# megvii-research/Far3D

Measured on AMD Instinct MI355X. Metric: samples/sec (7-cam frame) end-to-end @ VoV-99 640x960, higher is better.
Workload: dtype bf16x3; 1 GPU; BASELINE configs[1]: 7 cameras 3x640x960, VoV-99, A=1544 queries (644 learned + 644 adaptive + 256 propagated), 2312 self-attn keys, 6 decoder layers, streaming memory on, ego motion on; proposals=topk, fused_rows=True, parallelism=single GPU, weights=seeded random (far3d_amd.weights.init_state_dict, seed 0)

## Files before the change

### far3d_amd/csrc/conv_ws.hip

```cpp
#include "conv_ws.hpp"

#ifdef FAR3D_PROFILING
std::atomic<int> g_ws_ablate{0};
extern "C" int far3d_conv_ws_set_ablate(int mask) { g_ws_ablate.store(mask); return 0; }
#endif

int far3d_conv_ws_launch(const IgemmParams& P, int tile, hipStream_t st) {
  switch (tile) {
    case 400: return launch_conv3x3_ws<2, 4, 2, 2, 4, true, true>(P, st);
    case 401: return launch_conv3x3_ws<1, 8, 2, 1, 4, true, true>(P, st);
    case 402: return launch_conv3x3_ws<1, 8, 5, 1, 4, true, false>(P, st);
    case 403: return launch_conv3x3_ws<2, 4, 3, 1, 4, true, true>(P, st);
    case 404: return launch_conv3x3_ws<2, 2, 1, 2, 2, true, true>(P, st);
    case 405: return launch_conv3x3_ws<2, 4, 2, 1, 4, true, true>(P, st);
    case 406: return launch_conv3x3_ws<2, 4, 1, 2, 4, true, true>(P, st);
    case 407: return launch_conv3x3_ws<1, 4, 5, 1, 2, true, false>(P, st);
    case 408: return launch_conv3x3_ws<1, 4, 3, 1, 2, true, true>(P, st);
    case 409: return launch_conv3x3_ws<2, 4, 2, 2, 2, true, true>(P, st);
    case 410: return launch_conv3x3_ws<2, 4, 2, 2, 4, true, true, 4>(P, st);
    case 411: return launch_conv3x3_ws<2, 4, 2, 1, 4, true, true, 6>(P, st);
    case 412: return launch_conv3x3_ws<2, 4, 1, 2, 4, true, true, 8>(P, st);
    case 413: return launch_conv3x3_ws<1, 8, 2, 1, 4, true, true, 8>(P, st);
    case 414: return launch_conv3x3_ws<1, 4, 5, 1, 2, true, false, 5>(P, st);
    case 415: return launch_conv3x3_ws<2, 2, 1, 2, 2, true, true, 6>(P, st);
    case 416: return launch_conv3x3_ws<2, 4, 3, 1, 4, true, true, 4>(P, st);
    case 417: return launch_conv3x3_ws<2, 4, 2, 1, 4, true, true, 4>(P, st);
    case 418: return launch_conv3x3_ws<4, 2, 2, 2, 4, true, true, 3>(P, st);
    case 419: return launch_conv3x3_ws<4, 2, 2, 1, 4, true, true, 3>(P, st);
    case 440: return launch_conv3x3_ws<2, 4, 2, 2, 4, true, true, 3, true>(P, st);
    case 444: return launch_conv3x3_ws<2, 2, 1, 2, 2, true, true, 3, true>(P, st);
    case 445: return launch_conv3x3_ws<2, 4, 2, 1, 4, true, true, 6, true>(P, st);
    case 450: return launch_conv3x3_ws<2, 4, 2, 1, 4, true, true, 6, false, 3>(P, st);
    case 451: return launch_conv3x3_ws<2, 4, 1, 2, 4, true, true, 6, false, 3>(P, st);
    case 452: return launch_conv3x3_ws<2, 4, 1, 2, 4, true, true, 9, false, 3>(P, st);
    case 453: return launch_conv3x3_ws<1, 8, 2, 1, 4, true, true, 6, false, 3>(P, st);
    case 454: return launch_conv3x3_ws<1, 8, 2, 1, 4, true, true, 9, false, 3>(P, st);
    case 455: return launch_conv3x3_ws<1, 7, 2, 1, 4, true, true, 9, false, 3>(P, st);
    case 456: return launch_conv3x3_ws<2, 7, 1, 1, 2, true, true, 9, false, 3>(P, st);
    case 457: return launch_conv3x3_ws<2, 2, 1, 2, 2, true, true, 6, false, 3>(P, st);
    case 458: return launch_conv3x3_ws<1, 4, 3, 1, 2, true, true, 6, false, 3>(P, st);
    case 459: return launch_conv3x3_ws<2, 4, 1, 1, 4, true, true, 9, false, 3>(P, st);
    case 420: return launch_conv3x3_ws<2, 4, 2, 2, 4, false, true>(P, st);
    case 421: return launch_conv3x3_ws<1, 8, 2, 1, 4, false, true>(P, st);
    case 422: return launch_conv3x3_ws<1, 8, 5, 1, 4, false, true>(P, st);
    case 423: return launch_conv3x3_ws<2, 4, 3, 1, 4, false, true>(P, st);
    default: break;
  }
  far3d_set_error("far3d_conv2d_nhwc: unknown wave-specialised tile %d", tile);
  return FAR3D_ERR_ARG;
}

int far3d_gemm_ws_launch(const IgemmParams& P, int tile, hipStream_t st) {
  switch (tile) {
    case 460: return launch_gemm1x1_ws<4, 2, 1, 2, 4, 4, 1>(P, st);
    case 461: return launch_gemm1x1_ws<4, 2, 1, 2, 4, 4, 2>(P, st);
    case 462: return launch_gemm1x1_ws<2, 4, 2, 1, 4, 4, 2>(P, st);
    case 463: return launch_gemm1x1_ws<2, 2, 2, 2, 4, 4, 2>(P, st);
    case 464: return launch_gemm1x1_ws<4, 2, 2, 2, 4, 3, 1>(P, st);
    case 465: return launch_gemm1x1_ws<4, 2, 1, 2, 2, 4, 2>(P, st);
    case 466: return launch_gemm1x1_ws<2, 2, 1, 2, 4, 6, 3>(P, st);
    case 467: return launch_gemm1x1_ws<2, 4, 1, 1, 4, 6, 2>(P, st);
    case 468: return launch_gemm1x1_ws<2, 2, 1, 2, 2, 3, 1>(P, st);
    case 469: return launch_gemm1x1_ws<4, 2, 1, 2, 4, 2, 1>(P, st);
    case 470: return launch_gemm1x1_ws<2, 4, 2, 2, 4, 3, 1>(P, st);
    case 471: return launch_gemm1x1_ws<2, 2, 4, 2, 4, 3, 1>(P, st);
    case 473: return launch_gemm1x1_ws<4, 2, 2, 2, 2, 3, 1>(P, st);
    case 474: return launch_gemm1x1_ws<3, 2, 2, 2, 4, 3, 1>(P, st);
    case 475: return launch_gemm1x1_ws<2, 2, 2, 2, 4, 4, 1>(P, st);
    case 476: return launch_gemm1x1_ws<2, 4, 2, 2, 2, 3, 1>(P, st);
    default: break;
  }
  far3d_set_error("far3d_conv2d_nhwc: unknown wave-specialised GEMM tile %d", tile);
  return FAR3D_ERR_ARG;
}
```

### far3d_amd/csrc/conv_ws.hpp

```cpp
#pragma once
#include "igemm_kernels.hpp"
#include <type_traits>

__device__ __forceinline__ __amdgpu_buffer_rsrc_t uniform_rsrc(const void* p, long nbytes) {
  const unsigned long long a = (unsigned long long)(uintptr_t)p;
  const unsigned lo = __builtin_amdgcn_readfirstlane((unsigned)a), hi = __builtin_amdgcn_readfirstlane((unsigned)(a >> 32));
  const int nb = __builtin_amdgcn_readfirstlane((int)(nbytes < 0x7fffffffL ? nbytes : 0x7fffffffL));
  return __builtin_amdgcn_make_buffer_rsrc((void*)(uintptr_t)(((unsigned long long)hi << 32) | lo), 0, nb, 0x00020000);
}

__device__ __forceinline__ void wait_vmcnt_dyn(int n) {
#define FAR3D_WVC(k) case k: wait_vmcnt<k>(); break;
  switch (n) {
    FAR3D_WVC(0) FAR3D_WVC(1) FAR3D_WVC(2) FAR3D_WVC(3) FAR3D_WVC(4) FAR3D_WVC(5) FAR3D_WVC(6) FAR3D_WVC(7) FAR3D_WVC(8)
    FAR3D_WVC(9) FAR3D_WVC(10) FAR3D_WVC(11) FAR3D_WVC(12) FAR3D_WVC(13) FAR3D_WVC(14) FAR3D_WVC(15) FAR3D_WVC(16)
    FAR3D_WVC(17) FAR3D_WVC(18) FAR3D_WVC(19) FAR3D_WVC(20) FAR3D_WVC(21) FAR3D_WVC(22) FAR3D_WVC(23) FAR3D_WVC(24)
    FAR3D_WVC(25) FAR3D_WVC(26) FAR3D_WVC(27) FAR3D_WVC(28) FAR3D_WVC(29) FAR3D_WVC(30) FAR3D_WVC(31) FAR3D_WVC(32)
    FAR3D_WVC(33) FAR3D_WVC(34) FAR3D_WVC(35) FAR3D_WVC(36) FAR3D_WVC(37) FAR3D_WVC(38) FAR3D_WVC(39) FAR3D_WVC(40)
    FAR3D_WVC(41) FAR3D_WVC(42) FAR3D_WVC(43) FAR3D_WVC(44) FAR3D_WVC(45) FAR3D_WVC(46) FAR3D_WVC(47)
    default: wait_vmcnt<48>(); break;
  }
#undef FAR3D_WVC
}

#ifdef FAR3D_PROFILING
extern std::atomic<int> g_ws_ablate;
#define FAR3D_WS_ABLATE_ARG g_ws_ablate.load(std::memory_order_relaxed)
#else
#define FAR3D_WS_ABLATE_ARG 0
#endif

template <int WGM, int WGN, int WM, int WN, int NP, bool PAIR, bool DBUF, int NSW = 3, bool FLAGS = false, int GRP = 1>
__global__ __launch_bounds__(64 * (WGM * WGN + NP)) void conv3x3_ws_kernel(IgemmParams P, int tiles_x, int tiles_y, int n_mt, int n_items, int ablate) {
#if defined(__HIP_DEVICE_COMPILE__)
  constexpr int NWC = WGM * WGN;
  static_assert(NSW >= 3, "ring depth");
  static_assert(GRP == 1 || (GRP == 3 && (NSW == 6 || NSW == 9) && !FLAGS), "one barrier per tap, or per kernel row with a ring of 2 or 3 rows");
  constexpr int NG = NSW / GRP;
  constexpr int PLD = PAIR ? 2 : 1;
  constexpr int BM = 32 * WGM * WM, TH = WGN * WN, PW = 34, PH = TH + 2, PPIX = PW * PH;
  constexpr int PG = (PPIX + 15) / 16, PATCH_B = PG * 1024;
  constexpr int GA = BM / 16, WST = BM * 64, WSTAGE = PLD * WST;
  constexpr int PBASE = NSW * WSTAGE, PBUF = PLD * PATCH_B;
  constexpr int RB = WN + 2;
  constexpr int FLAGB = PBASE + 2 * PBUF;
  static_assert(FLAGB + (FLAGS ? 128 : 0) <= 163840, "LDS budget");
  static_assert(!FLAGS || (NP <= 4 && NWC <= 8), "flag words: one b128 read per 4 counters");
  extern __shared__ __attribute__((aligned(1024))) unsigned char smem[];
  [[maybe_unused]] volatile unsigned* const flg = reinterpret_cast<volatile unsigned*>(smem + FLAGB);
  if constexpr (FLAGS) {
    if (threadIdx.x < 32) flg[threadIdx.x] = 0u;
    __syncthreads();
  }
  [[maybe_unused]] bool gave_up = false;
  constexpr int SPIN_LIMIT = 1 << 18;
  const int t = threadIdx.x, lane = t & 63, wv = __builtin_amdgcn_readfirstlane(t >> 6);
  const int nchunks = P.cin_pad / 32;
  const int spt = 9 * nchunks;
  const int my_items = (n_items - (int)blockIdx.x + (int)gridDim.x - 1) / (int)gridDim.x;
  const int total_steps = my_items * spt, total_chunks = my_items * nchunks;
  const int Ktot = 9 * P.cin_pad * PLD;
#ifdef FAR3D_PROFILING
  if (P.prof && t == 0) {
    unsigned hw_, xcc_;
    asm volatile("s_getreg_b32 %0, hwreg(HW_REG_HW_ID)" : "=s"(hw_));
    asm volatile("s_getreg_b32 %0, hwreg(HW_REG_XCC_ID)" : "=s"(xcc_));
    P.prof[(long)blockIdx.x * 16 + 0] = (unsigned long long)hw_ | ((unsigned long long)xcc_ << 32);
    P.prof[(long)blockIdx.x * 16 + 6] = (unsigned long long)__builtin_amdgcn_s_memrealtime();
    P.prof[(long)blockIdx.x * 16 + 1] = (unsigned long long)__builtin_amdgcn_s_memtime();
    P.prof[(long)blockIdx.x * 16 + 4] = (unsigned long long)my_items;
  }
#endif

  if (wv >= NWC) {
    const int pw = wv - NWC;
    constexpr int GPL = (PG + NP - 1) / NP, GWL = (GA + NP - 1) / NP;
    const int rg = lane >> 2, pc = lane & 3;
    const int lc = pc ^ ((rg >> 2) & 3);
    int npq = (PG - pw + NP - 1) / NP, nwq = (GA - pw + NP - 1) / NP;
    npq = npq < 0 ? 0 : npq; nwq = nwq < 0 ? 0 : nwq;
    const int np = npq * PLD, nw = nwq * PLD;
    constexpr unsigned OOB = 0x80000000u;
    unsigned wvoff[GWL];
#pragma unroll
    for (int i = 0; i < GWL; ++i) wvoff[i] = (unsigned)((((pw + NP * i) * 16 + rg) * Ktot + lc * 8) * 2);
    const long img_bytes = (long)P.H * P.W * P.ldx * 2;
    unsigned pvoff[GPL];
    const bf16_t* x_base = nullptr;
    const bf16_t* w_base = nullptr;
    long w_bytes = 0;
    auto decode = [&](int k, int& n, int& y0, int& x0, int& m0) __attribute__((always_inline)) {
      const int item = (int)blockIdx.x + k * (int)gridDim.x;
      const int mt = item % n_mt, pt = item / n_mt;
      const int tx = pt % tiles_x, r = pt / tiles_x;
      const int ty = r % tiles_y;
      n = __builtin_amdgcn_readfirstlane(r / tiles_y); y0 = __builtin_amdgcn_readfirstlane(ty * TH);
      x0 = __builtin_amdgcn_readfirstlane(tx * 32); m0 = __builtin_amdgcn_readfirstlane(mt * BM);
    };
    auto set_w_tile = [&](int k) __attribute__((always_inline)) {
      int n, y0, x0, m0;
      decode(k, n, y0, x0, m0);
      w_base = reinterpret_cast<const bf16_t*>(P.w) + (long)m0 * Ktot;
      w_bytes = w_tile_bytes(BM, m0, P.Cout, Ktot);
    };
    auto set_p_tile = [&](int k) __attribute__((always_inline)) {
      int n, y0, x0, m0;
      decode(k, n, y0, x0, m0);
      x_base = reinterpret_cast<const bf16_t*>(P.x) + (long)n * P.x_img_stride;
#pragma unroll
      for (int i = 0; i < GPL; ++i) {
        const int idx = (pw + NP * i) * 16 + rg;
        const int py = idx / PW, px = idx - py * PW;
        const int iy = y0 - 1 + py, ix = x0 - 1 + px;
        const bool ok = idx < PPIX && iy >= 0 && iy < P.H && ix >= 0 && ix < P.W;
        pvoff[i] = ok ? (unsigned)((((long)iy * P.W + ix) * P.ldx + lc * 8) * 2) : OOB;
      }
    };
    auto issue_w = [&](int step_in_tile, int stage) __attribute__((always_inline)) {
      const int c = step_in_tile / 9, tap = step_in_tile - 9 * c;
      const int kb = __builtin_amdgcn_readfirstlane((tap * P.cin_pad + c * 32) * PLD * 2);
      const __amdgpu_buffer_rsrc_t rs_w = uniform_rsrc(w_base, w_bytes);
      const int sbase = __builtin_amdgcn_readfirstlane(stage * WSTAGE);
#pragma unroll
      for (int i = 0; i < GWL; ++i) {
        if (i < nwq) {
#pragma unroll
          for (int pl = 0; pl < PLD; ++pl)
            __builtin_amdgcn_raw_ptr_buffer_load_lds(rs_w, (lds_void_t*)(smem + sbase + pl * WST + (pw + NP * i) * 1024), 16, wvoff[i],
                                                     kb + pl * 64, 0, 0);
        }
      }
    };
    auto issue_p = [&](int chunk_in_tile, int buf) __attribute__((always_inline)) {
      const __amdgpu_buffer_rsrc_t rs_x = uniform_rsrc(x_base, img_bytes);
      const int pbase = __builtin_amdgcn_readfirstlane(PBASE + buf * PBUF), coff = __builtin_amdgcn_readfirstlane(chunk_in_tile * (64 * PLD));
#pragma unroll
      for (int i = 0; i < GPL; ++i) {
        if (i < npq) {
#pragma unroll
          for (int pl = 0; pl < PLD; ++pl)
            __builtin_amdgcn_raw_ptr_buffer_load_lds(rs_x, (lds_void_t*)(smem + pbase + pl * PATCH_B + (pw + NP * i) * 1024), 16, pvoff[i],
                                                     coff + pl * 64, 0, 0);
        }
      }
    };
    int sw_step = 0, sw_tile = 0, sw_stage = 0;
    int gp_chunk = 0, gp_tile = 0, gp_buf = 0;
    int w_left = total_steps, p_left = total_chunks;
    set_w_tile(0); set_p_tile(0);
    auto next_w = [&]() __attribute__((always_inline)) {
      if (!(ablate & 1)) issue_w(sw_step, sw_stage);
      --w_left;
      sw_stage = sw_stage == NSW - 1 ? 0 : sw_stage + 1;
      if (++sw_step == spt) { sw_step = 0; ++sw_tile; if (w_left > 0) set_w_tile(sw_tile); }
    };
    auto next_p = [&]() __attribute__((always_inline)) {
      if (!(ablate & 1)) issue_p(gp_chunk, gp_buf);
      --p_left;
      gp_buf ^= 1;
      if (++gp_chunk == nchunks) { gp_chunk = 0; ++gp_tile; if (p_left > 0) set_p_tile(gp_tile); }
    };
    next_p();
#pragma unroll
    for (int i = 0; i < (NG - 1) * GRP; ++i)
      if (w_left > 0) next_w();
    const int total_groups = total_steps / GRP, gpc = 9 / GRP;
    int gic = 0;
    unsigned phist = 0;
    for (int g = 0; g < total_groups; ++g) {
      int ahead = total_groups - 1 - g;
      ahead = ahead > NG - 2 ? NG - 2 : ahead;
      const int cnt = ahead * GRP * nw + __builtin_popcount(phist & ((1u << (NG - 1)) - 1u)) * np;
      const int S = g * GRP;
      if (ablate & 1) wait_vmcnt<0>(); else wait_vmcnt_dyn(cnt);
      if constexpr (FLAGS) {
        if (lane == 0) flg[pw] = (unsigned)(S + 1);
        if (S > 0 && !(ablate & 8)) {
          for (int spins = 0; !gave_up; ++spins) {
            const u32x4_t c0 = *reinterpret_cast<volatile u32x4_t*>(smem + FLAGB + 64);
            u32x4_t c1 = c0;
            if constexpr (NWC > 4) c1 = *reinterpret_cast<volatile u32x4_t*>(smem + FLAGB + 80);
            unsigned m = c0.x;
            if constexpr (NWC > 1) m = min(m, c0.y);
            if constexpr (NWC > 2) m = min(m, c0.z);
            if constexpr (NWC > 3) m = min(m, c0.w);
            if constexpr (NWC > 4) m = min(m, c1.x);
            if constexpr (NWC > 5) m = min(m, c1.y);
            if constexpr (NWC > 6) m = min(m, c1.z);
            if constexpr (NWC > 7) m = min(m, c1.w);
            if (__builtin_amdgcn_readfirstlane(m) >= (unsigned)S) break;
            if (spins > SPIN_LIMIT) gave_up = true;
            __builtin_amdgcn_s_sleep(2);
          }
        }
      } else {
#ifdef FAR3D_PROFILING
        if (!(ablate & 8))
#endif
        __builtin_amdgcn_s_barrier();
      }
      asm volatile("" ::: "memory");
#pragma unroll
      for (int i = 0; i < GRP; ++i)
        if (w_left > 0) next_w();
      phist <<= 1;
      if (gic == 0 && p_left > 0) { next_p(); phist |= 1u; }
      gic = gic == gpc - 1 ? 0 : gic + 1;
    }
    return;
  }

  const int wm = wv / WGN, wn = wv % WGN, l31 = lane & 31, hi = lane >> 5;
  int aaddr[WM], baddr[RB][3];
#pragma unroll
  for (int i = 0; i < WM; ++i) {
    const int r = (wm * WM + i) * 32 + l31;
    aaddr[i] = r * 64 + ((hi ^ ((r >> 2) & 3)) << 4);
  }
#pragma unroll
  for (int r = 0; r < RB; ++r)
#pragma unroll
    for (int kx = 0; kx < 3; ++kx) {
      const int idx = (wn * WN + r) * PW + l31 + kx;
      baddr[r][kx] = PBASE + idx * 64 + ((hi ^ ((idx >> 2) & 3)) << 4);
    }
  f32x16_t acc[WM][WN];
  u32x4_t fa[2][PLD][WM], fb[2][PLD][WN];

  auto load_a = [&](int set, int soff, int kk) __attribute__((always_inline)) {
#ifdef FAR3D_PROFILING
    if (ablate & 4) return;
#endif
    const int x32 = kk * 32;
#pragma unroll
    for (int pl = 0; pl < PLD; ++pl)
#pragma unroll
      for (int i = 0; i < WM; ++i) fa[set][pl][i] = *reinterpret_cast<const u32x4_t*>(smem + pl * WST + ((aaddr[i] ^ x32) + soff));
  };
  auto load_b = [&](int set, int tap, int kk) __attribute__((always_inline)) {
#ifdef FAR3D_PROFILING
    if (ablate & 4) return;
#endif
    const int ky = tap / 3, kx = tap - 3 * ky, x32 = kk * 32;
#pragma unroll
    for (int pl = 0; pl < PLD; ++pl)
#pragma unroll
      for (int j = 0; j < WN; ++j) fb[set][pl][j] = *reinterpret_cast<const u32x4_t*>(smem + pl * PATCH_B + (baddr[j + ky][kx] ^ x32));
  };
  auto load_set = [&](int set, int soff, int tap, int kk) __attribute__((always_inline)) { load_a(set, soff, kk); load_b(set, tap, kk); };
  auto mma_term = [&](int set, int term) __attribute__((always_inline)) {
    const int pa = (PAIR && term == 0) ? 1 : 0, pb = (PAIR && term == 1) ? 1 : 0;
#pragma unroll
    for (int i = 0; i < WM; ++i)
#pragma unroll
      for (int j = 0; j < WN; ++j) mma<bf16_t>(acc[i][j], fa[set][pa][i], fb[set][pb][j]);
  };
  auto mma_set = [&](int set) __attribute__((always_inline)) {
    if constexpr (PAIR) { mma_term(set, 0); mma_term(set, 1); }
    mma_term(set, 2);
  };

  int G = 0;
  int soff = 0;
  [[maybe_unused]] int Sg = 0;
  [[maybe_unused]] u32x4_t pfl = {0u, 0u, 0u, 0u};
#ifdef FAR3D_PROFILING
  unsigned long long pf_ta = 0, pf_tb = 0, pf_wait = 0, pf_body = 0, pf_epi = 0;
  const bool pf_on = P.prof != nullptr && wv == 0;
#endif
  for (int k = 0; k < my_items; ++k) {
    const int item = (int)blockIdx.x + k * (int)gridDim.x;
    const int mt = item % n_mt, pt = item / n_mt;
    const int tx = pt % tiles_x, rr = pt / tiles_x;
    const int ty = rr % tiles_y, n = rr / tiles_y;
    const int x0 = tx * 32, y0 = ty * TH, m0 = mt * BM;
#pragma unroll
    for (int i = 0; i < WM; ++i)
#pragma unroll
      for (int j = 0; j < WN; ++j)
#pragma unroll
        for (int r = 0; r < 16; ++r) acc[i][j][r] = 0.f;

    for (int c = 0; c < nchunks; ++c, ++G) {
#pragma unroll
      for (int tap = 0; tap < 9; ++tap) {
        const int stage = soff;
        if (tap % GRP == 0) {
        __builtin_amdgcn_s_waitcnt(0xc07f);
#ifdef FAR3D_PROFILING
        if (pf_on) {
          const unsigned long long now = __builtin_amdgcn_s_memtime();
          if (pf_tb) { pf_wait += pf_tb - pf_ta; pf_body += now - pf_tb; }
          pf_ta = now;
        }
#endif
        if constexpr (FLAGS) {
          if (lane == 0) flg[16 + wv] = (unsigned)Sg;
          if (!(ablate & 8)) {
            for (int spins = 0; !gave_up; ++spins) {
              unsigned m = pfl.x;
              if constexpr (NP > 1) m = min(m, pfl.y);
              if constexpr (NP > 2) m = min(m, pfl.z);
              if constexpr (NP > 3) m = min(m, pfl.w);
              if (__builtin_amdgcn_readfirstlane(m) >= (unsigned)(Sg + 1)) break;
              if (spins > SPIN_LIMIT) gave_up = true;
              __builtin_amdgcn_s_sleep(1);
              pfl = *reinterpret_cast<volatile u32x4_t*>(smem + FLAGB);
            }
          }
          ++Sg;
        } else {
#ifdef FAR3D_PROFILING
          if (!(ablate & 8))
#endif
          __builtin_amdgcn_s_barrier();
        }
        asm volatile("" ::: "memory");
        __builtin_amdgcn_sched_barrier(0);
#ifdef FAR3D_PROFILING
        if (pf_on) pf_tb = __builtin_amdgcn_s_memtime();
        if (tap == 0 && c == 0 && k == 0 && P.prof && t == 0) P.prof[(long)blockIdx.x * 16 + 2] = (unsigned long long)__builtin_amdgcn_s_memtime();
#endif
        }
        if (ablate & 2) { soff = soff == (NSW - 1) * WSTAGE ? 0 : soff + WSTAGE; continue; }
        if constexpr (DBUF) {
          load_set(0, stage, tap, 0);
          __builtin_amdgcn_sched_barrier(0);
          if (tap > 0 || c > 0) mma_set(1);
          __builtin_amdgcn_sched_barrier(0);
          load_a(1, stage, 1);
          if constexpr (FLAGS) pfl = *reinterpret_cast<volatile u32x4_t*>(smem + FLAGB);
          __builtin_amdgcn_sched_barrier(0);
          if constexpr (PAIR) {
            mma_term(0, 0);
            __builtin_amdgcn_sched_barrier(0);
            load_b(1, tap, 1);
            __builtin_amdgcn_sched_barrier(0);
            mma_term(0, 1);
            mma_term(0, 2);
          } else {
            load_b(1, tap, 1);
            __builtin_amdgcn_sched_barrier(0);
            mma_term(0, 2);
          }
          __builtin_amdgcn_sched_barrier(0);
          soff = soff == (NSW - 1) * WSTAGE ? 0 : soff + WSTAGE;
        } else {
          load_set(0, stage, tap, 0);
          __builtin_amdgcn_sched_barrier(0);
          mma_set(0);
          __builtin_amdgcn_sched_barrier(0);
          load_set(0, stage, tap, 1);
          if constexpr (FLAGS) pfl = *reinterpret_cast<volatile u32x4_t*>(smem + FLAGB);
          __builtin_amdgcn_sched_barrier(0);
          mma_set(0);
          __builtin_amdgcn_sched_barrier(0);
          soff = soff == (NSW - 1) * WSTAGE ? 0 : soff + WSTAGE;
        }
      }
      const int d = (G & 1) ? -PBUF : PBUF;
#pragma unroll
      for (int r = 0; r < RB; ++r)
#pragma unroll
        for (int kx = 0; kx < 3; ++kx) baddr[r][kx] += d;
    }
    if constexpr (DBUF) mma_set(1);
    __builtin_amdgcn_sched_barrier(0);
#ifdef FAR3D_PROFILING
    unsigned long long pf_e0 = 0;
    if (pf_on) {
      pf_e0 = __builtin_amdgcn_s_memtime();
      if (pf_tb) { pf_wait += pf_tb - pf_ta; pf_body += pf_e0 - pf_tb; pf_tb = 0; }
    }
#endif

    {
      const int px = x0 + l31;
      unsigned char* yb = reinterpret_cast<unsigned char*>(P.y);
#pragma unroll
      for (int j = 0; j < WN; ++j) {
        const int py = y0 + wn * WN + j;
        const bool ok = py < P.Ho && px < P.Wo;
        const long pix_b = ((long)n * P.y_img_stride + ((long)py * P.Wo + px) * P.ldy) * 2;
#pragma unroll
        for (int i = 0; i < WM; ++i) {
          const int cb = m0 + (wm * WM + i) * 32;
          if (cb >= P.Cout) continue;
#pragma unroll
          for (int qp = 0; qp < 2; ++qp) {
            uint2 h[2], l[2];
#pragma unroll
            for (int u = 0; u < 2; ++u) {
              const int q = 2 * qp + u;
              float4 b4 = make_float4(0.f, 0.f, 0.f, 0.f);
              if (P.bias) b4 = *reinterpret_cast<const float4*>(P.bias + cb + 8 * q + 4 * hi);
              float v[4];
#pragma unroll
              for (int e = 0; e < 4; ++e) v[e] = acc[i][j][4 * q + e];
              v[0] += b4.x; v[1] += b4.y; v[2] += b4.z; v[3] += b4.w;
              if (P.act == ACT_RELU) {
#pragma unroll
                for (int e = 0; e < 4; ++e) v[e] = fmaxf(v[e], 0.f);
              } else if (P.act == ACT_SWISH) {
                if constexpr (PAIR) {
#pragma unroll
                  for (int e = 0; e < 4; ++e) v[e] = v[e] * (1.f / (1.f + expf(-v[e])));
                } else {
#pragma unroll
                  for (int e = 0; e < 4; ++e) v[e] = v[e] * __frcp_rn(1.f + __expf(-v[e]));
                }
              }
              if constexpr (PAIR) split4f(v[0], v[1], v[2], v[3], h[u], l[u]);
              else { h[u] = make_uint2(pack_bf16x2(v[0], v[1]), pack_bf16x2(v[2], v[3])); l[u] = make_uint2(0u, 0u); }
            }
            u32x4_t oh, ol;
            {
              const auto sx = __builtin_amdgcn_permlane32_swap(h[0].x, h[1].x, false, false);
              const auto sy = __builtin_amdgcn_permlane32_swap(h[0].y, h[1].y, false, false);
              oh = u32x4_t{sx[0], sy[0], sx[1], sy[1]};
            }
            const int qoff = (2 * qp + hi) * 16;
            if constexpr (PAIR) {
              const auto sx = __builtin_amdgcn_permlane32_swap(l[0].x, l[1].x, false, false);
              const auto sy = __builtin_amdgcn_permlane32_swap(l[0].y, l[1].y, false, false);
              ol = u32x4_t{sx[0], sy[0], sx[1], sy[1]};
              if (ok) {
                unsigned char* d = yb + pix_b + (long)(cb >> 5) * 128 + qoff;
                *reinterpret_cast<u32x4_t*>(d) = oh;
                *reinterpret_cast<u32x4_t*>(d + 64) = ol;
              }
            } else {
              if (ok) *reinterpret_cast<u32x4_t*>(yb + pix_b + (long)cb * 2 + qoff) = oh;
            }
          }
        }
      }
    }
#ifdef FAR3D_PROFILING
    if (pf_on) pf_epi += __builtin_amdgcn_s_memtime() - pf_e0;
#endif
  }
#ifdef FAR3D_PROFILING
  if (P.prof && t == 0) {
    P.prof[(long)blockIdx.x * 16 + 3] = (unsigned long long)__builtin_amdgcn_s_memtime();
    P.prof[(long)blockIdx.x * 16 + 7] = (unsigned long long)__builtin_amdgcn_s_memrealtime();
    P.prof[(long)blockIdx.x * 16 + 5] = (unsigned long long)total_steps;
    P.prof[(long)blockIdx.x * 16 + 8] = pf_wait; P.prof[(long)blockIdx.x * 16 + 9] = pf_body; P.prof[(long)blockIdx.x * 16 + 10] = pf_epi;
  }
#endif
#endif
}

template <int WGM, int WGN, int WM, int WN, int NP, int NSW, int GRP, bool SUMS>
__global__ __launch_bounds__(64 * (WGM * WGN + NP)) void gemm1x1_ws_kernel(IgemmParams P, int npt, int nct, int ablate) {
#if defined(__HIP_DEVICE_COMPILE__)
  constexpr int NWC = WGM * WGN;
  constexpr int BM = 32 * WGM * WM, BP = 32 * WGN * WN;
  constexpr int GA = BM / 16, GB = BP / 16, SLOTS = GA + GB;
  static_assert(SLOTS % NP == 0, "every producer issues the same number of pieces per step (counted vmcnt)");
  constexpr int SPW = SLOTS / NP;
  constexpr int SUB = (BM + BP) * 64, STAGE = 2 * SUB;
  static_assert(NSW % GRP == 0 && NSW / GRP >= 2, "ring = at least two hand-over groups");
  constexpr int NG = NSW / GRP;
  extern __shared__ __attribute__((aligned(1024))) unsigned char smem[];
  const int t = threadIdx.x, lane = t & 63, wv = __builtin_amdgcn_readfirstlane(t >> 6);
  constexpr int SUMB = NSW * STAGE;
  static_assert(SUMB + 4 * BM * 8 <= 163840, "LDS budget");
  [[maybe_unused]] long long* const lsum = reinterpret_cast<long long*>(smem + SUMB);
  constexpr bool do_sums = SUMS;
  if (do_sums) {
    for (int i = threadIdx.x; i < 4 * BM; i += 64 * (NWC + NP)) lsum[i] = 0;
    __syncthreads();
  }
  const int HoWo = P.Ho * P.Wo;
  const long Npix = (long)P.N * HoWo;
  const int nsteps = P.cin_pad / 32;
  const int Ktot = P.cin_pad * 2;
  const int xcd = (int)blockIdx.x & 7, slot0 = (int)blockIdx.x >> 3, dslot = (int)gridDim.x >> 3;
  const int vslots = ((npt - xcd + 7) >> 3) * nct;
  const int my_items = vslots > slot0 ? (vslots - slot0 + dslot - 1) / dslot : 0;
  const int total_steps = my_items * nsteps;
  const int total_groups = (total_steps + GRP - 1) / GRP;
  auto decode = [&](int k, int& p0, int& m0) __attribute__((always_inline)) {
    const int slot = slot0 + k * dslot;
    const int ct = slot % nct, pt = (slot / nct) * 8 + xcd;
    p0 = __builtin_amdgcn_readfirstlane(pt * BP); m0 = __builtin_amdgcn_readfirstlane(ct * BM);
  };

  if (wv >= NWC) {
    const int pw = wv - NWC;
    const int rg = lane >> 2, pc = lane & 3;
    const int lc = pc ^ ((rg >> 2) & 3);
    constexpr unsigned OOB = 0x80000000u;
    const long x_bytes = ((long)(P.N - 1) * P.x_img_stride + (long)HoWo * P.ldx) * 2;
    unsigned voff[SPW];
    int sdst[SPW];
    bool isw[SPW];
#pragma unroll
    for (int i = 0; i < SPW; ++i) {
      const int q = pw + NP * i;
      isw[i] = q < GA;
      const int g = isw[i] ? q : q - GA;
      sdst[i] = (isw[i] ? 0 : BM * 64) + g * 1024;
      voff[i] = isw[i] ? (unsigned)(((g * 16 + rg) * Ktot + lc * 8) * 2) : 0u;
    }
    const bf16_t* w_base = nullptr;
    long w_bytes = 0;
    int cur_tile = 0, cur_step = 0, cur_stage = 0, left = total_steps;
    auto set_tile = [&](int k) __attribute__((always_inline)) {
      int p0, m0;
      decode(k, p0, m0);
      w_base = reinterpret_cast<const bf16_t*>(P.w) + (long)m0 * Ktot;
      w_bytes = w_tile_bytes(BM, m0, P.Cout, Ktot);
#pragma unroll
      for (int i = 0; i < SPW; ++i) {
        if (!isw[i]) {
          const int g = pw + NP * i - GA;
          const long p = (long)p0 + g * 16 + rg;
          if (p < Npix) {
            int n, rem;
            pix_split(p, HoWo, n, rem);
            voff[i] = (unsigned)(((long)n * P.x_img_stride + (long)rem * P.ldx + lc * 8) * 2);
          } else {
            voff[i] = OOB;
          }
        }
      }
    };
    auto next = [&]() __attribute__((always_inline)) {
      if (!(ablate & 1)) {
        const __amdgpu_buffer_rsrc_t rs_w = uniform_rsrc(w_base, w_bytes);
        const __amdgpu_buffer_rsrc_t rs_x = uniform_rsrc(P.x, x_bytes);
        const int sbase = __builtin_amdgcn_readfirstlane(cur_stage * STAGE);
        const int kb = __builtin_amdgcn_readfirstlane(cur_step * 128);
#pragma unroll
        for (int i = 0; i < SPW; ++i) {
#pragma unroll
          for (int pl = 0; pl < 2; ++pl) {
            if (isw[i])
              __builtin_amdgcn_raw_ptr_buffer_load_lds(rs_w, (lds_void_t*)(smem + sbase + pl * SUB + sdst[i]), 16, voff[i], kb + pl * 64, 0, 0);
            else
              __builtin_amdgcn_raw_ptr_buffer_load_lds(rs_x, (lds_void_t*)(smem + sbase + pl * SUB + sdst[i]), 16, voff[i], kb + pl * 64, 0, 0);
          }
        }
      }
      --left;
      cur_stage = cur_stage == NSW - 1 ? 0 : cur_stage + 1;
      if (++cur_step == nsteps) { cur_step = 0; ++cur_tile; if (left > 0) set_tile(cur_tile); }
    };
    if (my_items > 0) set_tile(0);
#pragma unroll
    for (int i = 0; i < (NG - 1) * GRP; ++i)
      if (left > 0) next();
    for (int g = 0; g < total_groups; ++g) {
      int later = total_steps - (g + 1) * GRP;
      later = later < 0 ? 0 : (later > (NG - 2) * GRP ? (NG - 2) * GRP : later);
      if (ablate & 1) wait_vmcnt<0>(); else wait_vmcnt_dyn(later * SPW * 2);
      __builtin_amdgcn_s_barrier();
      asm volatile("" ::: "memory");
#pragma unroll
      for (int i = 0; i < GRP; ++i)
        if (left > 0) next();
    }
    if (do_sums) __builtin_amdgcn_s_barrier();
    return;
  }

  const int wm = wv / WGN, wn = wv % WGN, l31 = lane & 31, hi = lane >> 5;
  int aaddr[WM], baddr[WN];
#pragma unroll
  for (int i = 0; i < WM; ++i) {
    const int r = (wm * WM + i) * 32 + l31;
    aaddr[i] = r * 64 + ((hi ^ ((r >> 2) & 3)) << 4);
  }
#pragma unroll
  for (int j = 0; j < WN; ++j) {
    const int r = (wn * WN + j) * 32 + l31;
    baddr[j] = BM * 64 + r * 64 + ((hi ^ ((r >> 2) & 3)) << 4);
  }
  f32x16_t acc[WM][WN];
  u32x4_t fa[2][2][WM], fb[2][2][WN];
  auto load_a = [&](int set, int soff, int kk) __attribute__((always_inline)) {
    const int x32 = kk * 32;
#pragma unroll
    for (int pl = 0; pl < 2; ++pl)
#pragma unroll
      for (int i = 0; i < WM; ++i) fa[set][pl][i] = *reinterpret_cast<const u32x4_t*>(smem + pl * SUB + ((aaddr[i] ^ x32) + soff));
  };
  auto load_b = [&](int set, int soff, int kk) __attribute__((always_inline)) {
    const int x32 = kk * 32;
#pragma unroll
    for (int pl = 0; pl < 2; ++pl)
#pragma unroll
      for (int j = 0; j < WN; ++j) fb[set][pl][j] = *reinterpret_cast<const u32x4_t*>(smem + pl * SUB + ((baddr[j] ^ x32) + soff));
  };
  auto mma_term = [&](int set, int term) __attribute__((always_inline)) {
    const int pa = term == 0 ? 1 : 0, pb = term == 1 ? 1 : 0;
#pragma unroll
    for (int i = 0; i < WM; ++i)
#pragma unroll
      for (int j = 0; j < WN; ++j) mma<bf16_t>(acc[i][j], fa[set][pa][i], fb[set][pb][j]);
  };
  int soff = 0, gs = 0;
  [[maybe_unused]] int flush_tile = 0, gcount = 0;
  auto flush = [&](int T) __attribute__((always_inline)) {
    int fp0, fm0;
    decode(T, fp0, fm0);
    const int fcam0 = (int)((long)fp0 / P.sums_hw);
    long long* src = lsum + (T & 1) * 2 * BM;
    for (int i = wv * 64 + lane; i < 2 * BM; i += 64 * NWC) {
      const int sl = i / BM, chn = i - sl * BM, cam = fcam0 + sl;
      const long long v = src[i];
      if (v != 0) {
        src[i] = 0;
        if (cam < P.N && fm0 + chn < P.Cout)
          atomicAdd(reinterpret_cast<unsigned long long*>(P.chan_sums + (long)cam * P.Cout + fm0 + chn), (unsigned long long)v);
      }
    }
  };
  for (int k = 0; k < my_items; ++k) {
    int p0, m0;
    decode(k, p0, m0);
#pragma unroll
    for (int i = 0; i < WM; ++i)
#pragma unroll
      for (int j = 0; j < WN; ++j)
#pragma unroll
        for (int r = 0; r < 16; ++r) acc[i][j][r] = 0.f;
    for (int s = 0; s < nsteps; ++s) {
      const int stage = soff;
      if (gs == 0) {
        __builtin_amdgcn_s_waitcnt(0xc07f);
        __builtin_amdgcn_s_barrier();
        asm volatile("" ::: "memory");
        __builtin_amdgcn_sched_barrier(0);
        if constexpr (do_sums) {
          while (flush_tile < k && ((flush_tile + 1) * nsteps - 1) / GRP < gcount) { flush(flush_tile); ++flush_tile; }
          ++gcount;
        }
      }
      gs = gs == GRP - 1 ? 0 : gs + 1;
      if (ablate & 2) { soff = soff == (NSW - 1) * STAGE ? 0 : soff + STAGE; continue; }
      load_a(0, stage, 0); load_b(0, stage, 0);
      __builtin_amdgcn_sched_barrier(0);
      if (s > 0) { mma_term(1, 0); mma_term(1, 1); mma_term(1, 2); }
      __builtin_amdgcn_sched_barrier(0);
      load_a(1, stage, 1);
      __builtin_amdgcn_sched_barrier(0);
      mma_term(0, 0);
      __builtin_amdgcn_sched_barrier(0);
      load_b(1, stage, 1);
      __builtin_amdgcn_sched_barrier(0);
      mma_term(0, 1);
      mma_term(0, 2);
      __builtin_amdgcn_sched_barrier(0);
      soff = soff == (NSW - 1) * STAGE ? 0 : soff + STAGE;
    }
    if (!(ablate & 2)) { mma_term(1, 0); mma_term(1, 1); mma_term(1, 2); }
    __builtin_amdgcn_sched_barrier(0);

    {
      unsigned char* yb = reinterpret_cast<unsigned char*>(P.y);
      const int cam0 = do_sums ? (int)((long)p0 / P.sums_hw) : 0;
      const long bnd = (long)(cam0 + 1) * P.sums_hw;
      const bool two = do_sums && (long)p0 + BP > bnd;
      long pix_b[WN];
      bool okj[WN], secj[WN];
#pragma unroll
      for (int j = 0; j < WN; ++j) {
        const long p = (long)p0 + (wn * WN + j) * 32 + l31;
        okj[j] = p < Npix;
        secj[j] = p >= bnd;
        pix_b[j] = 0;
        if (okj[j]) {
          int n, rem;
          pix_split(p, HoWo, n, rem);
          pix_b[j] = ((long)n * P.y_img_stride + (long)rem * P.ldy) * 2;
        }
      }
      auto stored = [&](int i, int j, int q, int cb, uint2& h, uint2& l) __attribute__((always_inline)) {
        float4 b4 = make_float4(0.f, 0.f, 0.f, 0.f);
        if (P.bias) b4 = *reinterpret_cast<const float4*>(P.bias + cb + 8 * q + 4 * hi);
        float v[4];
#pragma unroll
        for (int e = 0; e < 4; ++e) v[e] = acc[i][j][4 * q + e];
        v[0] += b4.x; v[1] += b4.y; v[2] += b4.z; v[3] += b4.w;
        if (P.act == ACT_RELU) {
#pragma unroll
          for (int e = 0; e < 4; ++e) v[e] = fmaxf(v[e], 0.f);
        } else if (P.act == ACT_SWISH) {
#pragma unroll
          for (int e = 0; e < 4; ++e) v[e] = v[e] * (1.f / (1.f + expf(-v[e])));
        }
        split4f(v[0], v[1], v[2], v[3], h, l);
      };
      auto quantise = [&](const uint2& h, const uint2& l, int q, int (&qs)[16], float& mx) __attribute__((always_inline)) {
        const unsigned w4[4] = {h.x, h.y, l.x, l.y};
#pragma unroll
        for (int e = 0; e < 2; ++e) {
          const float h0 = __uint_as_float(w4[e] << 16), h1 = __uint_as_float(w4[e] & 0xffff0000u);
          const float l0 = __uint_as_float(w4[2 + e] << 16), l1 = __uint_as_float(w4[2 + e] & 0xffff0000u);
          mx = fmaxf(mx, fmaxf(fabsf(h0), fabsf(h1)));
          qs[4 * q + 2 * e] += __float2int_rn(h0 * (float)(1 << FAR3D_SUMS_FRAC_BITS)) + __float2int_rn(l0 * (float)(1 << FAR3D_SUMS_FRAC_BITS));
          qs[4 * q + 2 * e + 1] += __float2int_rn(h1 * (float)(1 << FAR3D_SUMS_FRAC_BITS)) + __float2int_rn(l1 * (float)(1 << FAR3D_SUMS_FRAC_BITS));
        }
      };
      auto half_sum = [&](int x) __attribute__((always_inline)) -> int {
        x += __builtin_amdgcn_update_dpp(0, x, 0x128, 0xf, 0xf, true);
        x += __builtin_amdgcn_update_dpp(0, x, 0x124, 0xf, 0xf, true);
        x += __builtin_amdgcn_update_dpp(0, x, 0x122, 0xf, 0xf, true);
        x += __builtin_amdgcn_update_dpp(0, x, 0x121, 0xf, 0xf, true);
        typedef unsigned u2_t __attribute__((ext_vector_type(2)));
        const u2_t r = __builtin_amdgcn_permlane16_swap((unsigned)x, (unsigned)x, false, false);
        const unsigned rx = r.x, ry = r.y;
        return (int)(rx + ry);
      };
      auto reduce_add = [&](const int (&qs)[16], float mx, int sl, int cb) __attribute__((always_inline)) {
        const bool wide = WN > 2 || __any(mx >= (float)(1 << (24 - FAR3D_SUMS_FRAC_BITS)));
        long long* dst = lsum + ((k & 1) * 2 + sl) * BM + (cb - m0) + 4 * hi;
#pragma unroll
        for (int r = 0; r < 16; ++r) {
          long long tot;
          if (!wide) {
            tot = (long long)half_sum(qs[r]);
          } else {
            const int lo16 = qs[r] & 0xffff, hi16 = qs[r] >> 16;
            tot = (long long)half_sum(hi16) * 65536ll + (long long)half_sum(lo16);
          }
          if (l31 == 0 && tot != 0) atomicAdd(reinterpret_cast<unsigned long long*>(dst + 8 * (r >> 2) + (r & 3)), (unsigned long long)tot);
        }
      };
      auto channel_block = [&](auto ic) __attribute__((always_inline)) {
        constexpr int i = decltype(ic)::value;
        const int cb = m0 + (wm * WM + i) * 32;
        if (cb >= P.Cout) return;
        int qs[16];
        float mx = 0.f;
#pragma unroll
        for (int r = 0; r < 16; ++r) qs[r] = 0;
#pragma unroll
        for (int j = 0; j < WN; ++j) {
#pragma unroll
          for (int qp = 0; qp < 2; ++qp) {
            uint2 h[2], l[2];
#pragma unroll
            for (int u = 0; u < 2; ++u) {
              stored(i, j, 2 * qp + u, cb, h[u], l[u]);
              if (do_sums && okj[j] && !secj[j]) quantise(h[u], l[u], 2 * qp + u, qs, mx);
            }
            u32x4_t oh, ol;
            {
              const auto sx = __builtin_amdgcn_permlane32_swap(h[0].x, h[1].x, false, false);
              const auto sy = __builtin_amdgcn_permlane32_swap(h[0].y, h[1].y, false, false);
              oh = u32x4_t{sx[0], sy[0], sx[1], sy[1]};
            }
            {
              const auto sx = __builtin_amdgcn_permlane32_swap(l[0].x, l[1].x, false, false);
              const auto sy = __builtin_amdgcn_permlane32_swap(l[0].y, l[1].y, false, false);
              ol = u32x4_t{sx[0], sy[0], sx[1], sy[1]};
            }
            if (okj[j]) {
              unsigned char* d = yb + pix_b[j] + (long)(cb >> 5) * 128 + (2 * qp + hi) * 16;
              *reinterpret_cast<u32x4_t*>(d) = oh;
              *reinterpret_cast<u32x4_t*>(d + 64) = ol;
            }
          }
        }
        if constexpr (do_sums) {
          auto exact_add = [&](int sl) __attribute__((always_inline)) {
            long long* dst = lsum + ((k & 1) * 2 + sl) * BM + (cb - m0) + 4 * hi;
#pragma unroll
            for (int q = 0; q < 4; ++q) {
              long long x[4] = {0, 0, 0, 0};
#pragma unroll
              for (int j = 0; j < WN; ++j) {
                uint2 h, l;
                stored(i, j, q, cb, h, l);
                if (okj[j] && secj[j] == (sl == 1)) {
                  const unsigned w4[4] = {h.x, h.y, l.x, l.y};
#pragma unroll
                  for (int e = 0; e < 2; ++e) {
                    const float h0 = __uint_as_float(w4[e] << 16), h1 = __uint_as_float(w4[e] & 0xffff0000u);
                    const float l0 = __uint_as_float(w4[2 + e] << 16), l1 = __uint_as_float(w4[2 + e] & 0xffff0000u);
                    x[2 * e] += __double2ll_rn((double)h0 * (double)(1 << FAR3D_SUMS_FRAC_BITS)) + __double2ll_rn((double)l0 * (double)(1 << FAR3D_SUMS_FRAC_BITS));
                    x[2 * e + 1] += __double2ll_rn((double)h1 * (double)(1 << FAR3D_SUMS_FRAC_BITS)) + __double2ll_rn((double)l1 * (double)(1 << FAR3D_SUMS_FRAC_BITS));
                  }
                }
              }
#pragma unroll
              for (int e = 0; e < 4; ++e) {
                const long long v = x[e];
                const long long tot = (long long)half_sum((int)(v & 0xffff)) + ((long long)half_sum((int)((v >> 16) & 0xffff)) << 16) +
                                      ((long long)half_sum((int)((v >> 32) & 0xffff)) << 32) + ((long long)half_sum((int)(v >> 48)) << 48);
                if (l31 == 0 && tot != 0) atomicAdd(reinterpret_cast<unsigned long long*>(dst + 8 * q + e), (unsigned long long)tot);
              }
            }
          };
          const bool huge = __any(mx >= 2048.f);
          if (huge) exact_add(0); else reduce_add(qs, mx, 0, cb);
          if (two) {
            float mx1 = 0.f;
#pragma unroll
            for (int r = 0; r < 16; ++r) qs[r] = 0;
#pragma unroll
            for (int j = 0; j < WN; ++j)
#pragma unroll
              for (int q = 0; q < 4; ++q) {
                uint2 h, l;
                stored(i, j, q, cb, h, l);
                if (okj[j] && secj[j]) quantise(h, l, q, qs, mx1);
              }
            if (__any(mx1 >= 2048.f)) exact_add(1); else reduce_add(qs, mx1, 1, cb);
          }
        }
      };
      static_assert(WM <= 4, "channel blocks per consumer");
      channel_block(std::integral_constant<int, 0>{});
      if constexpr (WM > 1) channel_block(std::integral_constant<int, 1>{});
      if constexpr (WM > 2) channel_block(std::integral_constant<int, 2>{});
      if constexpr (WM > 3) channel_block(std::integral_constant<int, 3>{});
    }
  }
  if constexpr (do_sums) {
    __builtin_amdgcn_s_waitcnt(0xc07f);
    __builtin_amdgcn_s_barrier();
    asm volatile("" ::: "memory");
    while (flush_tile < my_items) { flush(flush_tile); ++flush_tile; }
  }
#endif
}

template <int WGM, int WGN, int WM, int WN, int NP, int NSW, int GRP>
static int launch_gemm1x1_ws(const IgemmParams& P, hipStream_t st) {
  constexpr int BM = 32 * WGM * WM, BP = 32 * WGN * WN;
  constexpr size_t lds = (size_t)NSW * 2 * (BM + BP) * 64 + 4 * BM * 8;
  static_assert(lds <= 163840, "LDS budget");
  const long Npix = (long)P.N * P.Ho * P.Wo;
  const int npt = (int)((Npix + BP - 1) / BP), nct = (P.Cout + BM - 1) / BM;
  static std::atomic<unsigned long long> lds_ok_s{0};
  static std::atomic<int> n_cu{0};
  int cus = n_cu.load(std::memory_order_relaxed);
  if (cus == 0) {
    int dev = 0;
    if (hipGetDevice(&dev) != hipSuccess) dev = 0;
    if (hipDeviceGetAttribute(&cus, hipDeviceAttributeMultiprocessorCount, dev) != hipSuccess || cus <= 0) cus = 256;
    n_cu.store(cus, std::memory_order_relaxed);
  }
  constexpr int wg_per_cu = lds <= 81920 && 64 * (WGM * WGN + NP) <= 1024 ? 2 : 1;
  const long items = (long)((npt + 7) / 8 * 8) * nct;
  long grid = (long)cus * wg_per_cu;
  grid = (grid + 7) / 8 * 8;
  if (items < grid) grid = items;
  static std::atomic<unsigned long long> lds_ok{0};
  if constexpr (lds > 65536)
    if (const int rc = far3d_allow_lds(P.chan_sums ? reinterpret_cast<const void*>(&gemm1x1_ws_kernel<WGM, WGN, WM, WN, NP, NSW, GRP, true>)
                                                   : reinterpret_cast<const void*>(&gemm1x1_ws_kernel<WGM, WGN, WM, WN, NP, NSW, GRP, false>),
                                       (int)lds, P.chan_sums ? lds_ok_s : lds_ok, "far3d_conv2d_nhwc")) return rc;
  if (P.chan_sums) {
    if (P.sums_hw < BP || P.cin_pad / 32 < 2 * GRP) {
      far3d_set_error("far3d_conv2d_nhwc: channel sums on this wave-specialised GEMM tile need Ho*Wo (%d) >= %d pixels and Cin >= %d", P.sums_hw, BP, 64 * GRP);
      return FAR3D_ERR_ARG;
    }
    hipLaunchKernelGGL((gemm1x1_ws_kernel<WGM, WGN, WM, WN, NP, NSW, GRP, true>), dim3((unsigned)grid), dim3(64 * (WGM * WGN + NP)), lds, st, P, npt, nct, FAR3D_WS_ABLATE_ARG);
  } else {
    hipLaunchKernelGGL((gemm1x1_ws_kernel<WGM, WGN, WM, WN, NP, NSW, GRP, false>), dim3((unsigned)grid), dim3(64 * (WGM * WGN + NP)), lds, st, P, npt, nct, FAR3D_WS_ABLATE_ARG);
  }
  return 0;
}

template <int WGM, int WGN, int WM, int WN, int NP, bool PAIR, bool DBUF, int NSW = 3, bool FLAGS = false, int GRP = 1>
static int launch_conv3x3_ws(const IgemmParams& P, hipStream_t st) {
  constexpr int BM = 32 * WGM * WM, TH = WGN * WN, PLD = PAIR ? 2 : 1;
  constexpr int PG = (34 * (TH + 2) + 15) / 16;
  constexpr size_t lds = (size_t)NSW * PLD * BM * 64 + (size_t)2 * PLD * PG * 1024 + (FLAGS ? 128 : 0);
  static_assert(lds <= 163840, "LDS budget");
  const int tiles_x = (P.Wo + 31) / 32, tiles_y = (P.Ho + TH - 1) / TH, n_mt = (P.Cout + BM - 1) / BM;
  const int n_items = P.N * tiles_x * tiles_y * n_mt;
  static std::atomic<int> n_cu{0};
  int cus = n_cu.load(std::memory_order_relaxed);
  if (cus == 0) {
    int dev = 0;
    if (hipGetDevice(&dev) != hipSuccess) dev = 0;
    if (hipDeviceGetAttribute(&cus, hipDeviceAttributeMultiprocessorCount, dev) != hipSuccess || cus <= 0) cus = 256;
    n_cu.store(cus, std::memory_order_relaxed);
  }
  constexpr int wg_per_cu = lds <= 81920 && 64 * (WGM * WGN + NP) <= 1024 ? 2 : 1;
  const int grid = n_items < cus * wg_per_cu ? n_items : cus * wg_per_cu;
  static std::atomic<unsigned long long> lds_ok{0};
  if constexpr (lds > 65536)
    if (const int rc = far3d_allow_lds(reinterpret_cast<const void*>(&conv3x3_ws_kernel<WGM, WGN, WM, WN, NP, PAIR, DBUF, NSW, FLAGS, GRP>), (int)lds, lds_ok, "far3d_conv2d_nhwc")) return rc;
  hipLaunchKernelGGL((conv3x3_ws_kernel<WGM, WGN, WM, WN, NP, PAIR, DBUF, NSW, FLAGS, GRP>), dim3((unsigned)grid), dim3(64 * (WGM * WGN + NP)), lds, st, P, tiles_x, tiles_y, n_mt,
                     n_items, FAR3D_WS_ABLATE_ARG);
  return 0;
}
```

Before: 72.02 samples/s.

## Add configurable pixel-tile width to wave-specialised 3x3 conv kernel

Adds a TW template parameter so a 3x3 conv block can cover tiles of arbitrary width (whole rows of TW pixels) instead of fixed 32-wide rows, with per-tap LDS patch addresses precomputed per fragment and the epilogue mapping pixels through the new tiling. It also registers six new tile variants using wider tiles. The aim is to fit feature maps whose width is not a multiple of 32 and to improve patch halo reuse. The cost is more address registers (9 per fragment), and the new variants only take effect if the tile selector picks them.

```diff
diff --git a/far3d_amd/csrc/conv_ws.hip b/far3d_amd/csrc/conv_ws.hip
--- a/far3d_amd/csrc/conv_ws.hip
+++ b/far3d_amd/csrc/conv_ws.hip
@@ -40,6 +40,12 @@
     case 457: return launch_conv3x3_ws<2, 2, 1, 2, 2, true, true, 6, false, 3>(P, st);
     case 458: return launch_conv3x3_ws<1, 4, 3, 1, 2, true, true, 6, false, 3>(P, st);
     case 459: return launch_conv3x3_ws<2, 4, 1, 1, 4, true, true, 9, false, 3>(P, st);
+    case 441: return launch_conv3x3_ws<4, 3, 1, 1, 4, true, true, 6, false, 3, 12>(P, st);
+    case 442: return launch_conv3x3_ws<4, 3, 1, 1, 4, true, true, 6, false, 3, 24>(P, st);
+    case 443: return launch_conv3x3_ws<2, 6, 1, 1, 4, true, true, 6, false, 3, 24>(P, st);
+    case 446: return launch_conv3x3_ws<5, 3, 1, 1, 1, true, true, 6, false, 3, 12>(P, st);
+    case 447: return launch_conv3x3_ws<3, 5, 1, 1, 1, true, true, 6, false, 3, 20>(P, st);
+    case 448: return launch_conv3x3_ws<5, 3, 1, 1, 1, true, true, 6, false, 3, 24>(P, st);
     case 420: return launch_conv3x3_ws<2, 4, 2, 2, 4, false, true>(P, st);
     case 421: return launch_conv3x3_ws<1, 8, 2, 1, 4, false, true>(P, st);
     case 422: return launch_conv3x3_ws<1, 8, 5, 1, 4, false, true>(P, st);
diff --git a/far3d_amd/csrc/conv_ws.hpp b/far3d_amd/csrc/conv_ws.hpp
--- a/far3d_amd/csrc/conv_ws.hpp
+++ b/far3d_amd/csrc/conv_ws.hpp
@@ -30,7 +30,7 @@
 #define FAR3D_WS_ABLATE_ARG 0
 #endif
 
-template <int WGM, int WGN, int WM, int WN, int NP, bool PAIR, bool DBUF, int NSW = 3, bool FLAGS = false, int GRP = 1>
+template <int WGM, int WGN, int WM, int WN, int NP, bool PAIR, bool DBUF, int NSW = 3, bool FLAGS = false, int GRP = 1, int TW = 0>
 __global__ __launch_bounds__(64 * (WGM * WGN + NP)) void conv3x3_ws_kernel(IgemmParams P, int tiles_x, int tiles_y, int n_mt, int n_items, int ablate) {
 #if defined(__HIP_DEVICE_COMPILE__)
   constexpr int NWC = WGM * WGN;
@@ -38,7 +38,9 @@
   static_assert(GRP == 1 || (GRP == 3 && (NSW == 6 || NSW == 9) && !FLAGS), "one barrier per tap, or per kernel row with a ring of 2 or 3 rows");
   constexpr int NG = NSW / GRP;
   constexpr int PLD = PAIR ? 2 : 1;
-  constexpr int BM = 32 * WGM * WM, TH = WGN * WN, PW = 34, PH = TH + 2, PPIX = PW * PH;
+  static_assert(TW == 0 || (TW >= 2 && (32 * WGN * WN) % TW == 0), "a block is whole rows of TW pixels");
+  constexpr int BW = TW > 0 ? TW : 32;
+  constexpr int BM = 32 * WGM * WM, TH = TW > 0 ? 32 * WGN * WN / TW : WGN * WN, PW = BW + 2, PH = TH + 2, PPIX = PW * PH;
   constexpr int PG = (PPIX + 15) / 16, PATCH_B = PG * 1024;
   constexpr int GA = BM / 16, WST = BM * 64, WSTAGE = PLD * WST;
   constexpr int PBASE = NSW * WSTAGE, PBUF = PLD * PATCH_B;
@@ -95,7 +97,7 @@
       const int tx = pt % tiles_x, r = pt / tiles_x;
       const int ty = r % tiles_y;
       n = __builtin_amdgcn_readfirstlane(r / tiles_y); y0 = __builtin_amdgcn_readfirstlane(ty * TH);
-      x0 = __builtin_amdgcn_readfirstlane(tx * 32); m0 = __builtin_amdgcn_readfirstlane(mt * BM);
+      x0 = __builtin_amdgcn_readfirstlane(tx * BW); m0 = __builtin_amdgcn_readfirstlane(mt * BM);
     };
     auto set_w_tile = [&](int k) __attribute__((always_inline)) {
       int n, y0, x0, m0;
@@ -211,19 +213,33 @@
   }
 
   const int wm = wv / WGN, wn = wv % WGN, l31 = lane & 31, hi = lane >> 5;
-  int aaddr[WM], baddr[RB][3];
+  int aaddr[WM];
+  constexpr int BA0 = TW > 0 ? WN : RB, BA1 = TW > 0 ? 9 : 3;
+  int baddr[BA0][BA1];
 #pragma unroll
   for (int i = 0; i < WM; ++i) {
     const int r = (wm * WM + i) * 32 + l31;
     aaddr[i] = r * 64 + ((hi ^ ((r >> 2) & 3)) << 4);
   }
-#pragma unroll
-  for (int r = 0; r < RB; ++r)
-#pragma unroll
-    for (int kx = 0; kx < 3; ++kx) {
-      const int idx = (wn * WN + r) * PW + l31 + kx;
-      baddr[r][kx] = PBASE + idx * 64 + ((hi ^ ((idx >> 2) & 3)) << 4);
-    }
+  if constexpr (TW > 0) {
+#pragma unroll
+    for (int j = 0; j < WN; ++j) {
+      const int p = (wn * WN + j) * 32 + l31, py = p / TW, px = p - py * TW;
+#pragma unroll
+      for (int tap = 0; tap < 9; ++tap) {
+        const int idx = (py + tap / 3) * PW + px + tap % 3;
+        baddr[j][tap] = PBASE + idx * 64 + ((hi ^ ((idx >> 2) & 3)) << 4);
+      }
+    }
+  } else {
+#pragma unroll
+    for (int r = 0; r < RB; ++r)
+#pragma unroll
+      for (int kx = 0; kx < 3; ++kx) {
+        const int idx = (wn * WN + r) * PW + l31 + kx;
+        baddr[r][kx] = PBASE + idx * 64 + ((hi ^ ((idx >> 2) & 3)) << 4);
+      }
+  }
   f32x16_t acc[WM][WN];
   u32x4_t fa[2][PLD][WM], fb[2][PLD][WN];
 
@@ -245,7 +261,10 @@
 #pragma unroll
     for (int pl = 0; pl < PLD; ++pl)
 #pragma unroll
-      for (int j = 0; j < WN; ++j) fb[set][pl][j] = *reinterpret_cast<const u32x4_t*>(smem + pl * PATCH_B + (baddr[j + ky][kx] ^ x32));
+      for (int j = 0; j < WN; ++j) {
+        const int ba = TW > 0 ? baddr[j][tap] : baddr[j + ky][kx];
+        fb[set][pl][j] = *reinterpret_cast<const u32x4_t*>(smem + pl * PATCH_B + (ba ^ x32));
+      }
   };
   auto load_set = [&](int set, int soff, int tap, int kk) __attribute__((always_inline)) { load_a(set, soff, kk); load_b(set, tap, kk); };
   auto mma_term = [&](int set, int term) __attribute__((always_inline)) {
@@ -273,7 +292,7 @@
     const int mt = item % n_mt, pt = item / n_mt;
     const int tx = pt % tiles_x, rr = pt / tiles_x;
     const int ty = rr % tiles_y, n = rr / tiles_y;
-    const int x0 = tx * 32, y0 = ty * TH, m0 = mt * BM;
+    const int x0 = tx * BW, y0 = ty * TH, m0 = mt * BM;
 #pragma unroll
     for (int i = 0; i < WM; ++i)
 #pragma unroll
@@ -360,9 +379,9 @@
       }
       const int d = (G & 1) ? -PBUF : PBUF;
 #pragma unroll
-      for (int r = 0; r < RB; ++r)
-#pragma unroll
-        for (int kx = 0; kx < 3; ++kx) baddr[r][kx] += d;
+      for (int r = 0; r < BA0; ++r)
+#pragma unroll
+        for (int kx = 0; kx < BA1; ++kx) baddr[r][kx] += d;
     }
     if constexpr (DBUF) mma_set(1);
     __builtin_amdgcn_sched_barrier(0);
@@ -375,11 +394,11 @@
 #endif
 
     {
-      const int px = x0 + l31;
       unsigned char* yb = reinterpret_cast<unsigned char*>(P.y);
 #pragma unroll
       for (int j = 0; j < WN; ++j) {
-        const int py = y0 + wn * WN + j;
+        const int bp = (wn * WN + j) * 32 + l31;
+        const int py = y0 + (TW > 0 ? bp / BW : wn * WN + j), px = x0 + (TW > 0 ? bp % BW : l31);
         const bool ok = py < P.Ho && px < P.Wo;
         const long pix_b = ((long)n * P.y_img_stride + ((long)py * P.Wo + px) * P.ldy) * 2;
 #pragma unroll
@@ -868,13 +887,14 @@
   return 0;
 }
 
-template <int WGM, int WGN, int WM, int WN, int NP, bool PAIR, bool DBUF, int NSW = 3, bool FLAGS = false, int GRP = 1>
+template <int WGM, int WGN, int WM, int WN, int NP, bool PAIR, bool DBUF, int NSW = 3, bool FLAGS = false, int GRP = 1, int TW = 0>
 static int launch_conv3x3_ws(const IgemmParams& P, hipStream_t st) {
-  constexpr int BM = 32 * WGM * WM, TH = WGN * WN, PLD = PAIR ? 2 : 1;
-  constexpr int PG = (34 * (TH + 2) + 15) / 16;
+  constexpr int BW = TW > 0 ? TW : 32;
+  constexpr int BM = 32 * WGM * WM, TH = TW > 0 ? 32 * WGN * WN / TW : WGN * WN, PLD = PAIR ? 2 : 1;
+  constexpr int PG = ((BW + 2) * (TH + 2) + 15) / 16;
   constexpr size_t lds = (size_t)NSW * PLD * BM * 64 + (size_t)2 * PLD * PG * 1024 + (FLAGS ? 128 : 0);
   static_assert(lds <= 163840, "LDS budget");
-  const int tiles_x = (P.Wo + 31) / 32, tiles_y = (P.Ho + TH - 1) / TH, n_mt = (P.Cout + BM - 1) / BM;
+  const int tiles_x = (P.Wo + BW - 1) / BW, tiles_y = (P.Ho + TH - 1) / TH, n_mt = (P.Cout + BM - 1) / BM;
   const int n_items = P.N * tiles_x * tiles_y * n_mt;
   static std::atomic<int> n_cu{0};
   int cus = n_cu.load(std::memory_order_relaxed);
@@ -888,8 +908,8 @@
   const int grid = n_items < cus * wg_per_cu ? n_items : cus * wg_per_cu;
   static std::atomic<unsigned long long> lds_ok{0};
   if constexpr (lds > 65536)
-    if (const int rc = far3d_allow_lds(reinterpret_cast<const void*>(&conv3x3_ws_kernel<WGM, WGN, WM, WN, NP, PAIR, DBUF, NSW, FLAGS, GRP>), (int)lds, lds_ok, "far3d_conv2d_nhwc")) return rc;
-  hipLaunchKernelGGL((conv3x3_ws_kernel<WGM, WGN, WM, WN, NP, PAIR, DBUF, NSW, FLAGS, GRP>), dim3((unsigned)grid), dim3(64 * (WGM * WGN + NP)), lds, st, P, tiles_x, tiles_y, n_mt,
+    if (const int rc = far3d_allow_lds(reinterpret_cast<const void*>(&conv3x3_ws_kernel<WGM, WGN, WM, WN, NP, PAIR, DBUF, NSW, FLAGS, GRP, TW>), (int)lds, lds_ok, "far3d_conv2d_nhwc")) return rc;
+  hipLaunchKernelGGL((conv3x3_ws_kernel<WGM, WGN, WM, WN, NP, PAIR, DBUF, NSW, FLAGS, GRP, TW>), dim3((unsigned)grid), dim3(64 * (WGM * WGN + NP)), lds, st, P, tiles_x, tiles_y, n_mt,
                      n_items, FAR3D_WS_ABLATE_ARG);
   return 0;
 }
```

Result: faster. 72.89 samples/s, median of 6 (+1.2%).
